# wizardyesterday/RtlSdrDiags

Measured on AMD Instinct MI355X. Metric: IQ MSamples/s through WBFM chain at 1/2/4/8 GPUs; % HBM roofline, higher is better.
Workload: dtype int8/int16 Q15 + f32; 1 GPU; BASELINE configs[1]: WBFM, 1 channel, 2^28-sample synthetic IQ; channels_per_gpu=1, log2_samples_per_channel=28, kernels=streaming pipelines

## Files before the change

### rtlsdrdiags_amd/csrc/iqd_stream_fix.h

```cpp
#pragma once
#include <hip/hip_runtime.h>

#include "iqd_kernels.h"
#include "iqd_stream.h"
#include "iqd_stream_mixed.h"
#include "iqd_wbfm.h"
#include "iqd_mfma.h"

namespace iqd {

struct StSeg {
    uint32_t valid, li, tile, ch, ech;
    int32_t v0, tlen;
    int32_t vlen;
};

__device__ __forceinline__ StSeg st_segment(const ChainLaunch &a, uint32_t sid, uint32_t n_segments)
{
    StSeg s;
    s.valid = sid < n_segments ? 1u : 0u;
    const uint32_t id = s.valid ? sid : 0u;
    s.li = id / a.tiles_per_ch;
    s.tile = id - s.li * a.tiles_per_ch;
    s.ch = a.ch_list[s.li];
    s.ech = a.first_ch + s.ch;
    const uint32_t vlen = a.vlen_gated ? a.vlen_gated[s.ch] : a.vlen;
    s.vlen = (int32_t)vlen;
    const int64_t v0 = (int64_t)s.tile * a.tile_len;
    if (v0 >= (int64_t)vlen) { s.valid = 0; s.v0 = 0; s.tlen = 0; return s; }
    s.v0 = (int32_t)v0;
    const int64_t rest = (int64_t)vlen - v0;
    s.tlen = (int32_t)(rest < (int64_t)a.tile_len ? rest : (int64_t)a.tile_len);
    if (!s.valid) s.tlen = 0;
    return s;
}

#ifndef IQD_ST_NO_GROUPS
#define IQD_ST_NO_GROUPS 0
#endif
__device__ __forceinline__ StSeg st_segment_of(const ChainLaunch &a, const StreamArgs &sa, uint32_t sid, int &rot)
{
    if (IQD_ST_NO_GROUPS || !sa.grouped) { rot = 0; return st_segment(a, sid, sa.n_segments); }
    const uint32_t r = (sid >= sa.group_start[1] ? 1u : 0u) + (sid >= sa.group_start[2] ? 1u : 0u);
    rot = 1 - (int)r;
    const uint32_t local = sid - sa.group_start[r];
    const bool there = sid < sa.group_start[3] && local < sa.group_nseg[r];
    return st_segment(a, there ? sa.group_li0[r] * a.tiles_per_ch + local : sa.n_segments, sa.n_segments);
}
__device__ __forceinline__ uint32_t st_id_count(const StreamArgs &sa) { return !IQD_ST_NO_GROUPS && sa.grouped ? sa.group_start[3] : sa.n_segments; }

#ifndef IQD_FIX_LANES
#define IQD_FIX_LANES 16
#endif
constexpr int FIX_LANES = IQD_FIX_LANES;
constexpr int FIX_SEGS = 256 / FIX_LANES;
constexpr int FIX_THREADS = FIX_LANES * FIX_SEGS;
static_assert(FIX_LANES == 16 || FIX_LANES == 32, "threads per boundary");
struct FixLds {
    uint32_t rec[(FIX_SEGS + 1) * 64];
    uint32_t y2x[FIX_SEGS][41];
};
__device__ __forceinline__ void wbfm_stream_fixup_body(const ChainLaunch &a, const StreamArgs &sa, const uint32_t block, FixLds &fl)
{
    uint32_t (&rec)[(FIX_SEGS + 1) * 64] = fl.rec;
    uint32_t (&y2x)[FIX_SEGS][41] = fl.y2x;
    const uint32_t sid0 = block * FIX_SEGS;
    const int tid = (int)threadIdx.x, sl = tid / FIX_LANES, i = tid % FIX_LANES;
    const uint32_t sid = sid0 + (uint32_t)sl;
    const StSeg sg = st_segment(a, sid < sa.n_segments ? sid : 0u, sa.n_segments);
    const bool live = sid < sa.n_segments && sg.valid && sg.tile != 0;
    float y_in = 0.f, y_end = 0.f;
    if (live && i == FIX_LANES - 1) {
        const WbfmRecord *r = a.records + (size_t)sg.li * a.tiles_per_ch;
        y_in = r[sg.tile].y_in;
        y_end = r[sg.tile - 1].y_end;
    }
    {
        const uint32_t *src = (const uint32_t *)sa.hist + ((size_t)sid0 - (sid0 ? 1 : 0)) * 64;
        const uint32_t n_avail = (sa.n_segments - sid0 < (uint32_t)FIX_SEGS ? sa.n_segments - sid0 : (uint32_t)FIX_SEGS) + (sid0 ? 1u : 0u);
        for (uint32_t k = (uint32_t)tid; k < n_avail * 64; k += FIX_THREADS) rec[k + (sid0 ? 0 : 64)] = src[k];
    }
    __syncthreads();
    const StHist &prev = *(const StHist *)&rec[sl * 64], &own = *(const StHist *)&rec[(sl + 1) * 64];
    if (live && i < 3) {
        int acc = 1 << 14;
        acc = dot2(prev.w_last[0], sa.d1p[0], acc);
        acc = dot2(prev.w_last[1], sa.d1p[1], acc);
        acc = dot2(own.w_first[0], sa.d1p[2], acc);
        acc = dot2(own.w_first[1], sa.d1p[3], acc);
        uint32_t y1[10];
#pragma unroll
        for (int k = 0; k < 4; k++) y1[k] = prev.y1_last[k];
#pragma unroll
        for (int k = 0; k < 6; k++) y1[4 + k] = own.y1_first[k];
        y1[4] = (y1[4] & 0xffff0000u) | ((uint32_t)(acc >> 15) & 0xffffu);
        int s2 = 1 << 14;
#pragma unroll
        for (int q = 0; q < 6; q++) {
            const uint32_t d = i == 0 ? y1[5 - q] : (i == 1 ? y1[7 - q] : y1[9 - q]);
            s2 = dot2(d, sa.p12p[q], s2);
        }
        ((int16_t *)&y2x[sl][20])[i] = (int16_t)(s2 >> 15);
    } else if (live) {
        for (int p = i - 3; p < 41; p += FIX_LANES - 3) {
            if (p == 20) continue;
            if (p == 21) ((int16_t *)&y2x[sl][21])[1] = (int16_t)(own.y2_first[1] >> 16);
            else y2x[sl][p] = p < 20 ? prev.y2_last[p] : own.y2_first[p - 20];
        }
    }
    if (live && i == FIX_LANES - 1 && f2u(y_in) != f2u(y_end)) {
        if (!iir_states_agree(y_in, y_end, a.params[sg.ech].wbfm_k >= 1.0f)) {
            atomicAdd(&a.counters[CNT_TILE_MISMATCH], 1u);
            atomicAdd(&a.counters[CNT_STREAM_MISMATCH], 1u);
            a.repair_flags[sg.li] = 1;
        }
    }
    __syncthreads();
    if (!live) return;
    for (int j = i; j < ST_FIX_PCM && j < sg.tlen / 32; j += FIX_LANES) {
        int s3 = 1 << 14;
#pragma unroll
        for (int q = 0; q < 20; q++) {
            const uint32_t pair = y2x[sl][20 + j - q];
            s3 = clamp_q30(dot2(pair, sa.a40p[q] & 0xffff0000u, s3));
            s3 = clamp_q30(dot2(pair, sa.a40p[q] & 0x0000ffffu, s3));
        }
        a.pcm[(size_t)sg.ch * a.pcm_stride + (sg.v0 >> 5) + j] = (int16_t)(s3 >> 15);
    }
}

}
```

Measured before the change: 875,700 MSamples/s.

## Vectorize fixup history loads, overlap them with segment math, skip clamps when quiet

The fixup kernel now issues 16-byte vector loads of the history records into registers first. It then computes the segment descriptor and reads the IIR records while those loads are in flight, and only afterwards stores the values into LDS, so global latency overlaps with the scalar work. The 40-tap audio FIR tail gains a per-boundary ballot that checks whether every sample stays below a safe amplitude. If so, it uses one unclamped dot2 per tap pair instead of two clamped half-dots. This adds an alignment requirement on the LDS union, extra registers for the staged loads, and a correctness dependence on the AUDIO40_SAFE bound.

Result: faster. 888,400 MSamples/s, median of 6 (+1.4%).

```diff
diff --git a/rtlsdrdiags_amd/csrc/iqd_stream_fix.h b/rtlsdrdiags_amd/csrc/iqd_stream_fix.h
--- a/rtlsdrdiags_amd/csrc/iqd_stream_fix.h
+++ b/rtlsdrdiags_amd/csrc/iqd_stream_fix.h
@@ -57,9 +57,10 @@
 constexpr int FIX_THREADS = FIX_LANES * FIX_SEGS;
 static_assert(FIX_LANES == 16 || FIX_LANES == 32, "threads per boundary");
 struct FixLds {
-    uint32_t rec[(FIX_SEGS + 1) * 64];
+    alignas(16) uint32_t rec[(FIX_SEGS + 1) * 64];
     uint32_t y2x[FIX_SEGS][41];
 };
+static_assert(sizeof(FixLds) == ((FIX_SEGS + 1) * 64 + FIX_SEGS * 41) * 4, "the alignment adds no padding (a union member of mixed_tail_kernel's LDS)");
 __device__ __forceinline__ void wbfm_stream_fixup_body(const ChainLaunch &a, const StreamArgs &sa, const uint32_t block, FixLds &fl)
 {
     uint32_t (&rec)[(FIX_SEGS + 1) * 64] = fl.rec;
@@ -67,18 +68,45 @@
     const uint32_t sid0 = block * FIX_SEGS;
     const int tid = (int)threadIdx.x, sl = tid / FIX_LANES, i = tid % FIX_LANES;
     const uint32_t sid = sid0 + (uint32_t)sl;
-    const StSeg sg = st_segment(a, sid < sa.n_segments ? sid : 0u, sa.n_segments);
-    const bool live = sid < sa.n_segments && sg.valid && sg.tile != 0;
+    const bool there = sid < sa.n_segments;
+    StSeg sg;
+    sg.li = (there ? sid : 0u) / a.tiles_per_ch;
+    sg.tile = (there ? sid : 0u) - sg.li * a.tiles_per_ch;
+    constexpr int REC16 = (FIX_SEGS + 1) * 16, TRIPS = (REC16 + FIX_THREADS - 1) / FIX_THREADS;
+    const uint32_t n_avail = (sa.n_segments - sid0 < (uint32_t)FIX_SEGS ? sa.n_segments - sid0 : (uint32_t)FIX_SEGS) + (sid0 ? 1u : 0u);
+    const uint32_t n16 = n_avail * 16;
+    v4u t[TRIPS];
+    {
+        const v4u *src = (const v4u *)sa.hist + ((size_t)sid0 - (sid0 ? 1 : 0)) * 16;
+#pragma unroll
+        for (int k = 0; k < TRIPS; k++) {
+            const uint32_t k16 = (uint32_t)(tid + k * FIX_THREADS);
+            t[k] = src[k16 < n16 ? k16 : n16 - 1];
+        }
+    }
     float y_in = 0.f, y_end = 0.f;
-    if (live && i == FIX_LANES - 1) {
+    if (i == FIX_LANES - 1) {
         const WbfmRecord *r = a.records + (size_t)sg.li * a.tiles_per_ch;
         y_in = r[sg.tile].y_in;
-        y_end = r[sg.tile - 1].y_end;
+        y_end = r[sg.tile ? sg.tile - 1 : 0].y_end;
     }
+    sg.ch = a.ch_list[sg.li];
+    sg.ech = a.first_ch + sg.ch;
+    sg.vlen = (int32_t)(a.vlen_gated ? a.vlen_gated[sg.ch] : a.vlen);
     {
-        const uint32_t *src = (const uint32_t *)sa.hist + ((size_t)sid0 - (sid0 ? 1 : 0)) * 64;
-        const uint32_t n_avail = (sa.n_segments - sid0 < (uint32_t)FIX_SEGS ? sa.n_segments - sid0 : (uint32_t)FIX_SEGS) + (sid0 ? 1u : 0u);
-        for (uint32_t k = (uint32_t)tid; k < n_avail * 64; k += FIX_THREADS) rec[k + (sid0 ? 0 : 64)] = src[k];
+        const int64_t v0 = (int64_t)sg.tile * a.tile_len, rest = (int64_t)(uint32_t)sg.vlen - v0;
+        sg.valid = there && rest > 0 ? 1u : 0u;
+        sg.v0 = sg.valid ? (int32_t)v0 : 0;
+        sg.tlen = !sg.valid ? 0 : (int32_t)(rest < (int64_t)a.tile_len ? rest : (int64_t)a.tile_len);
+    }
+    const bool live = sg.valid && sg.tile != 0;
+    static_assert(TRIPS == 1 || TRIPS == 2, "one statement names all of a thread's loads: one wait");
+    if constexpr (TRIPS == 2) asm volatile("" : "+v"(t[0]), "+v"(t[TRIPS - 1]));
+    else asm volatile("" : "+v"(t[0]));
+#pragma unroll
+    for (int k = 0; k < TRIPS; k++) {
+        const uint32_t k16 = (uint32_t)(tid + k * FIX_THREADS);
+        if (k16 < n16) ((v4u *)rec)[k16 + (sid0 ? 0 : 16)] = t[k];
     }
     __syncthreads();
     const StHist &prev = *(const StHist *)&rec[sl * 64], &own = *(const StHist *)&rec[(sl + 1) * 64];
@@ -117,15 +145,39 @@
     }
     __syncthreads();
     if (!live) return;
-    for (int j = i; j < ST_FIX_PCM && j < sg.tlen / 32; j += FIX_LANES) {
-        int s3 = 1 << 14;
+    bool loud_lane = false;
+    for (int p = i; p < 41; p += FIX_LANES) {
+        const uint32_t pair = y2x[sl][p];
+        const int lo = (int)(pair << 16) >> 16, hi = (int)pair >> 16;
+        loud_lane |= (uint32_t)(lo < 0 ? -lo : lo) > (uint32_t)AUDIO40_SAFE || (uint32_t)(hi < 0 ? -hi : hi) > (uint32_t)AUDIO40_SAFE;
+    }
+    const uint64_t lanes_of_boundary = (FIX_LANES == 32 ? 0xffffffffull : 0xffffull) << ((tid & 63) / FIX_LANES * FIX_LANES);
+    const bool quiet = (__ballot(loud_lane) & lanes_of_boundary) == 0;
+    int16_t *pcm = a.pcm + (size_t)sg.ch * a.pcm_stride + (sg.v0 >> 5);
+    if (quiet) {
+        for (int j = i; j < ST_FIX_PCM && j < sg.tlen / 32; j += FIX_LANES) {
+            int s3 = 1 << 14;
+#pragma unroll
+            for (int q = 0; q < 20; q++) s3 = dot2(y2x[sl][20 + j - q], sa.a40p[q], s3);
+            pcm[j] = (int16_t)(s3 >> 15);
+        }
+    } else {
+        uint32_t newer[20], older[20];
 #pragma unroll
         for (int q = 0; q < 20; q++) {
-            const uint32_t pair = y2x[sl][20 + j - q];
-            s3 = clamp_q30(dot2(pair, sa.a40p[q] & 0xffff0000u, s3));
-            s3 = clamp_q30(dot2(pair, sa.a40p[q] & 0x0000ffffu, s3));
+            newer[q] = (uint32_t)__builtin_amdgcn_readfirstlane((int)(sa.a40p[q] & 0xffff0000u));
+            older[q] = (uint32_t)__builtin_amdgcn_readfirstlane((int)(sa.a40p[q] & 0x0000ffffu));
         }
-        a.pcm[(size_t)sg.ch * a.pcm_stride + (sg.v0 >> 5) + j] = (int16_t)(s3 >> 15);
+        for (int j = i; j < ST_FIX_PCM && j < sg.tlen / 32; j += FIX_LANES) {
+            int s3 = 1 << 14;
+#pragma unroll
+            for (int q = 0; q < 20; q++) {
+                const uint32_t pair = y2x[sl][20 + j - q];
+                s3 = clamp_q30(dot2(pair, newer[q], s3));
+                s3 = clamp_q30(dot2(pair, older[q], s3));
+            }
+            pcm[j] = (int16_t)(s3 >> 15);
+        }
     }
 }
 
```
